# f4ah6o/duckdb.mbt

Measured on NVIDIA B200. Metric: datachunk_to_arrow_rows_per_s, higher is better.
Workload: dtype u8

## Files before the change

duckdb.mbt_b200/csrc/dmb_common.cuh:

```cuda
#pragma once

#include <cuda_runtime.h>
#include <stdint.h>

#include "duckdb_mb_gpu.h"

namespace dmb {

constexpr int kThreads = 256;
constexpr int kVec = DMB_VECTOR_SIZE;
constexpr int kNumSMs = 148;

void set_error(const char *fmt, ...);
int32_t check_cuda(cudaError_t e, const char *what);

struct alignas(16) i128 {
  uint64_t lo;
  int64_t hi;
};
struct alignas(16) u128 {
  uint64_t lo;
  uint64_t hi;
};
struct alignas(16) interval_t {
  int32_t months;
  int32_t days;
  int64_t micros;
};
struct alignas(16) month_day_nano_t {
  int32_t months;
  int32_t days;
  int64_t nanos;
};

template <typename T, int R>
struct alignas(sizeof(T) * R) Pack {
  T v[R];
};

template <int N>
struct RawVec;
template <>
struct RawVec<1> { using type = unsigned char; };
template <>
struct RawVec<2> { using type = unsigned short; };
template <>
struct RawVec<4> { using type = unsigned int; };
template <>
struct RawVec<8> { using type = uint2; };
template <>
struct RawVec<16> { using type = uint4; };

template <typename P>
__device__ __forceinline__ P ld_stream(const P *p) {
  using R = typename RawVec<sizeof(P)>::type;
  R r = __ldcs(reinterpret_cast<const R *>(p));
  P out;
  memcpy(&out, &r, sizeof(P));
  return out;
}
template <typename P>
__device__ __forceinline__ void st_stream(P *p, const P &v) {
  using R = typename RawVec<sizeof(P)>::type;
  R r;
  memcpy(&r, &v, sizeof(P));
  __stcs(reinterpret_cast<R *>(p), r);
}

struct BatchView {
  const uint32_t *counts;
  const int64_t *row_off;
  int64_t nchunks;
  int64_t nrows;
};

__device__ __forceinline__ int64_t find_chunk(const BatchView &b, int64_t row) {
  int64_t lo = 0, hi = b.nchunks;
  while (hi - lo > 1) {
    int64_t mid = (lo + hi) >> 1;
    if (__ldg(b.row_off + mid) <= row) lo = mid; else hi = mid;
  }
  return lo;
}

__device__ __forceinline__ uint64_t chunk_valid_bits(const uint64_t *vslab, const dmb_vec_desc *vecs,
                                                     int64_t c, int local, int take) {
  uint64_t keep = take >= 64 ? ~0ull : ((1ull << take) - 1ull);
  int64_t vo = vecs[c].val_off;
  if (vo < 0) return keep;
  const uint64_t *m = vslab + vo;
  int w = local >> 6, s = local & 63;
  uint64_t bits = __ldg(m + w) >> s;
  if (s && s + take > 64) bits |= __ldg(m + w + 1) << (64 - s);
  return bits & keep;
}

__device__ __forceinline__ uint64_t gather_valid64(const BatchView &b, const uint64_t *vslab,
                                                   const dmb_vec_desc *vecs, int64_t r0) {
  if (r0 >= b.nrows) return 0ull;
  int64_t c = find_chunk(b, r0);
  uint64_t word = 0;
  int filled = 0;
  while (filled < 64 && r0 + filled < b.nrows) {
    int64_t local = r0 + filled - __ldg(b.row_off + c);
    int64_t avail = (int64_t)__ldg(b.counts + c) - local;
    if (avail <= 0) { ++c; continue; }
    int take = (int)(avail < (int64_t)(64 - filled) ? avail : (int64_t)(64 - filled));
    word |= chunk_valid_bits(vslab, vecs, c, (int)local, take) << filled;
    filled += take;
  }
  return word;
}

__device__ __forceinline__ bool tile_is_regular(const BatchView &b, int64_t t) {
  if (t >= b.nchunks) return false;
  int64_t ro = __ldg(b.row_off + t);
  if (ro != t * (int64_t)kVec) return false;
  uint32_t cnt = __ldg(b.counts + t);
  return cnt == (uint32_t)kVec || ro + cnt == b.nrows;
}

__device__ __forceinline__ uint32_t pack8(uint64_t bytes01) {
  return (uint32_t)((bytes01 * 0x0102040810204080ull) >> 56);
}
__device__ __forceinline__ uint64_t spread8(uint32_t bits) {
  uint64_t x = (uint64_t)(bits & 0xff) * 0x0101010101010101ull;
  x &= 0x8040201008040201ull;
  x += 0x7f7f7f7f7f7f7f7full;
  return (x >> 7) & 0x0101010101010101ull;
}

struct BitSrc {
  const uint32_t *w;
  int64_t base;
};
__device__ __forceinline__ BitSrc bit_src(const uint8_t *bm, int64_t bit_offset) {
  const uintptr_t a = reinterpret_cast<uintptr_t>(bm);
  return BitSrc{reinterpret_cast<const uint32_t *>(a & ~(uintptr_t)3), bit_offset + (int64_t)(a & 3u) * 8};
}

__device__ __forceinline__ uint32_t load_bits32(const uint32_t *w, int64_t p, int take) {
  const int64_t wi = p >> 5;
  const int s = (int)(p & 31);
  const uint32_t lo = __ldg(w + wi);
  const uint32_t hi = (s + take > 32) ? __ldg(w + wi + 1) : 0u;
  const uint32_t r = __funnelshift_r(lo, hi, (uint32_t)s);
  return take >= 32 ? r : (r & ((1u << take) - 1u));
}

__device__ __forceinline__ uint4 shift_words(const uint4 &a, const uint4 &b, int ws, uint32_t sh) {
  uint32_t w0, w1, w2, w3, w4;
  switch (ws) {
    case 0: w0 = a.x; w1 = a.y; w2 = a.z; w3 = a.w; w4 = b.x; break;
    case 1: w0 = a.y; w1 = a.z; w2 = a.w; w3 = b.x; w4 = b.y; break;
    case 2: w0 = a.z; w1 = a.w; w2 = b.x; w3 = b.y; w4 = b.z; break;
    default: w0 = a.w; w1 = b.x; w2 = b.y; w3 = b.z; w4 = b.w; break;
  }
  return make_uint4(__funnelshift_r(w0, w1, sh), __funnelshift_r(w1, w2, sh), __funnelshift_r(w2, w3, sh), __funnelshift_r(w3, w4, sh));
}

template <int W>
__device__ __forceinline__ uint32_t word_keep(uint32_t bits, int i) {
  if (W >= 4) return ((bits >> (i * 4 / W)) & 1u) ? 0xffffffffu : 0u;
  if (W == 2) {
    const uint32_t b = bits >> (2 * i);
    return ((b & 1u) ? 0x0000ffffu : 0u) | ((b & 2u) ? 0xffff0000u : 0u);
  }
  const uint32_t b = bits >> (4 * i);
  return ((b & 1u) | ((b & 2u) << 7) | ((b & 4u) << 14) | ((b & 8u) << 21)) * 0xffu;
}

__device__ __forceinline__ uint4 enum_entry(const dmb_enum_job &job, uint32_t idx) {
  const uint32_t o0 = __ldg(job.dict_offsets + idx), o1 = __ldg(job.dict_offsets + idx + 1);
  const uint32_t len = o1 - o0;
  const uint8_t *q = job.dict_data + o0;
  uint4 e = make_uint4(len, 0, 0, 0);
  if (len <= 12u) {
    uint32_t w[3] = {0u, 0u, 0u};
#pragma unroll
    for (uint32_t k = 0; k < 12u; ++k)
      if (k < len) w[k >> 2] |= (uint32_t)__ldg(q + k) << (8u * (k & 3u));
    e.y = w[0]; e.z = w[1]; e.w = w[2];
  } else {
    e.y = (uint32_t)__ldg(q) | ((uint32_t)__ldg(q + 1) << 8) | ((uint32_t)__ldg(q + 2) << 16) | ((uint32_t)__ldg(q + 3) << 24);
    const uint64_t p = job.dict_host_base + o0;
    e.z = (uint32_t)p;
    e.w = (uint32_t)(p >> 32);
  }
  return e;
}


constexpr uint64_t kFlagAggregate = 1ull << 62;
constexpr uint64_t kFlagPrefix = 2ull << 62;
constexpr uint64_t kValueMask = (1ull << 62) - 1ull;
__device__ __forceinline__ uint64_t ld_status(const unsigned long long *p) {
  return *reinterpret_cast<const volatile unsigned long long *>(p);
}
__device__ __forceinline__ unsigned long long global_ns() { unsigned long long t; asm volatile("mov.u64 %0, %globaltimer;" : "=l"(t)); return t; }

constexpr unsigned long long kGroupOne = 1ull << 56;
constexpr unsigned long long kGroupSumMask = kGroupOne - 1ull;
__device__ __forceinline__ uint64_t lookback_groups(const unsigned long long *status, const unsigned long long *gsum, const unsigned long long *gpre,
                                                    int64_t tile, int lane, unsigned long long *err_flags, unsigned long long err_bit,
                                                    unsigned long long limit_ns) {
  if (tile <= 0) return 0;
  const int64_t g = tile >> 5;
  const int64_t lo = g >= 1 ? 32 * (g - 1) : 0;
  const int64_t idx0 = tile - 1 - lane, idx1 = tile - 33 - lane;
  const bool in0 = idx0 >= lo, in1 = idx1 >= lo;
  int64_t hbase = g - 2;
  uint64_t st0 = 0, st1 = 0, ga = 0, gb = 0;
  uint64_t prefix = 0;
  unsigned long long t0 = 0;
  unsigned spins = 0;
  auto give_up = [&]() -> bool {
    ++spins;
    if (spins > 8u) __nanosleep(100);
    if ((spins & 63u) != 0u && limit_ns != 0ull) return false;
    const unsigned long long now = global_ns();
    if (t0 == 0) t0 = now;
    if (__any_sync(0xffffffffu, now - t0 > limit_ns)) {
      if (lane == 0) atomicOr(err_flags, err_bit);
      return true;
    }
    return false;
  };
  {
    const int64_t h = hbase - lane;
    if (h >= 0) { ga = ld_status(gpre + h); gb = ld_status(gsum + h); }
  }
  {
    uint64_t v;
    int state;
    while (true) {
      if (in0 && (st0 >> 62) == 0) st0 = ld_status(status + idx0);
      if (in1 && (st1 >> 62) == 0) st1 = ld_status(status + idx1);
      v = 0;
      state = 0;
#pragma unroll
      for (int j = 0; j < 2; ++j) {
        const uint64_t st = j ? st1 : st0;
        const bool in = j ? in1 : in0;
        if (state == 0) {
          const uint32_t ready = __ballot_sync(0xffffffffu, !in || (st >> 62) != 0);
          const uint32_t is_p = __ballot_sync(0xffffffffu, in && (st >> 62) == 2);
          const int first_p = is_p ? (__ffs(is_p) - 1) : 31;
          const uint32_t need = first_p >= 31 ? 0xffffffffu : ((2u << first_p) - 1u);
          if ((ready & need) != need) state = 2;
          else {
            if (in && lane <= first_p) v += st & kValueMask;
            if (is_p) state = 1;
          }
        }
      }
      if (state != 2) break;
      if (give_up()) { state = 1; break; }
    }
#pragma unroll
    for (int d = 16; d > 0; d >>= 1) v += __shfl_xor_sync(0xffffffffu, v, d);
    prefix = v;
    if (state == 1) return prefix;
  }
  while (true) {
    const int64_t h = hbase - lane;
    uint32_t is_p;
    int first_p;
    while (true) {
      const bool pa = h < 0 || (ga >> 62) == 2;
      const bool cb = h >= 0 && ((gb >> 56) & 63ull) == 32ull;
      is_p = __ballot_sync(0xffffffffu, pa);
      first_p = is_p ? (__ffs(is_p) - 1) : 32;
// ... 21 lines not shown
```

duckdb.mbt_b200/csrc/kernels_fixed.cu:

```cuda

#include "dmb_common.cuh"

namespace dmb {

constexpr int kGroupU = 4;

template <typename S>
__device__ __forceinline__ int64_t to_i64(S v) { return (int64_t)v; }
template <>
__device__ __forceinline__ int64_t to_i64<uint64_t>(uint64_t v) {
  return v > 0x7fffffffffffffffull ? 0 : (int64_t)v;
}
template <>
__device__ __forceinline__ int64_t to_i64<double>(double v) {
  if (!(v >= -9223372036854775808.0 && v < 9223372036854775808.0)) return 0;
  return __double2ll_rn(v);
}
template <>
__device__ __forceinline__ int64_t to_i64<float>(float v) {
  if (!(v >= -9223372036854775808.0f && v < 9223372036854775808.0f)) return 0;
  return __float2ll_rn(v);
}
template <>
__device__ __forceinline__ int64_t to_i64<i128>(i128 v) {
// ... 59 lines not shown
  const __int128 q = (x + rounding) / power;
  return (q >= -(__int128)9223372036854775807ll - 1 && q <= (__int128)9223372036854775807ll) ? (int64_t)q : 0;
}
template <typename S>
__device__ __forceinline__ double dec_to_f64(S v, int scale) {
  const int64_t x = (int64_t)v;
  const double dp = kDoublePow10[scale < 0 ? 0 : (scale > 38 ? 38 : scale)];
  if (scale == 0 || (x <= 9007199254740992ll && x >= -9007199254740992ll)) return (double)x / dp;
  const int64_t power = pow10_i64(scale);
  return (double)(x / power) + (double)(x % power) / dp;
}
template <>
__device__ __forceinline__ double dec_to_f64<i128>(i128 v, int scale) {
  const __int128 x = as_int128(v);
  const double dp = kDoublePow10[scale < 0 ? 0 : (scale > 38 ? 38 : scale)];
  if (scale == 0 || (x <= (__int128)9007199254740992ll && x >= -(__int128)9007199254740992ll)) return int128_to_f64(x) / dp;
  const __int128 power = pow10_i128(scale);
  return int128_to_f64(x / power) + int128_to_f64(x % power) / dp;
}

template <typename S>
__device__ __forceinline__ int32_t to_i32_sat(S v) {
  int64_t x = (int64_t)v;
  return x > 2147483647ll ? 2147483647 : (x < -2147483648ll ? (int32_t)-2147483648ll : (int32_t)x);
}
template <>
__device__ __forceinline__ int32_t to_i32_sat<uint64_t>(uint64_t v) {
  return v > 2147483647ull ? 2147483647 : (int32_t)v;
}

__device__ __forceinline__ int64_t floor_div(int64_t a, int64_t b) {
  int64_t q = a / b;
  return (a % b != 0 && ((a < 0) != (b < 0))) ? q - 1 : q;
}

__device__ __forceinline__ int32_t date_ref_quirk(int32_t days) {
  int64_t z = (int64_t)days + 719468;
  int64_t era = (z >= 0 ? z : z - 146096) / 146097;
  int64_t doe = z - era * 146097;
  int64_t yoe = (doe - doe / 1460 + doe / 36524 - doe / 146096) / 365;
  int64_t y = yoe + era * 400;
  int64_t doy = doe - (365 * yoe + yoe / 4 - yoe / 100);
  int64_t mp = (5 * doy + 2) / 153;
  int64_t m = mp < 10 ? mp + 3 : mp - 9;
  if (m <= 2) y += 1;
  if (y >= 1970 || y < 1 || y > 9999) return days;
  auto leaps_before = [](int64_t yy) { return yy / 4 - yy / 100 + yy / 400; };
  int64_t missing = leaps_before(1969) - leaps_before(y - 1);
  return (int32_t)((int64_t)days + missing);
}

struct CvNoParam { __device__ __forceinline__ CvNoParam(int32_t = 0) {} };
struct CvSame : CvNoParam { using CvNoParam::CvNoParam; template <typename S> __device__ __forceinline__ S operator()(S v) const { return v; } };
struct CvI64 : CvNoParam { using CvNoParam::CvNoParam; template <typename S> __device__ __forceinline__ int64_t operator()(S v) const { return to_i64<S>(v); } };
struct CvI32Trunc : CvNoParam { using CvNoParam::CvNoParam; template <typename S> __device__ __forceinline__ int32_t operator()(S v) const { return (int32_t)to_i64<S>(v); } };
struct CvF64 : CvNoParam { using CvNoParam::CvNoParam; template <typename S> __device__ __forceinline__ double operator()(S v) const { return to_f64<S>(v); } };
struct CvBoolByte : CvNoParam { using CvNoParam::CvNoParam; template <typename S> __device__ __forceinline__ uint8_t operator()(S v) const { return nonzero<S>(v) ? 1 : 0; } };
struct CvI32Sat : CvNoParam { using CvNoParam::CvNoParam; template <typename S> __device__ __forceinline__ int32_t operator()(S v) const { return to_i32_sat<S>(v); } };
struct CvDecBase { int scale; __device__ __forceinline__ CvDecBase(int32_t p = 0) : scale(p) {} };
struct CvDecI64 : CvDecBase { using CvDecBase::CvDecBase; template <typename S> __device__ __forceinline__ int64_t operator()(S v) const { return dec_to_i64<S>(v, scale); } };
struct CvDecI32Trunc : CvDecBase { using CvDecBase::CvDecBase; template <typename S> __device__ __forceinline__ int32_t operator()(S v) const { return (int32_t)dec_to_i64<S>(v, scale); } };
struct CvDecF64 : CvDecBase { using CvDecBase::CvDecBase; template <typename S> __device__ __forceinline__ double operator()(S v) const { return dec_to_f64<S>(v, scale); } };
struct CvDecBoolByte : CvDecBase { using CvDecBase::CvDecBase; template <typename S> __device__ __forceinline__ uint8_t operator()(S v) const { return dec_to_i64<S>(v, scale) != 0 ? 1 : 0; } };
struct CvI128 : CvNoParam {
  using CvNoParam::CvNoParam;
  template <typename S> __device__ __forceinline__ i128 operator()(S v) const {
    i128 r; r.lo = (uint64_t)(int64_t)v; r.hi = (int64_t)v < 0 ? -1 : 0; return r;
  }
};
struct CvTsS : CvNoParam { using CvNoParam::CvNoParam; __device__ __forceinline__ int64_t operator()(int64_t v) const { return (int64_t)((uint64_t)v * 1000000ull); } };
struct CvTsMs : CvNoParam { using CvNoParam::CvNoParam; __device__ __forceinline__ int64_t operator()(int64_t v) const { return (int64_t)((uint64_t)v * 1000ull); } };
struct CvTsNs : CvNoParam { using CvNoParam::CvNoParam; __device__ __forceinline__ int64_t operator()(int64_t v) const { return floor_div(v, 1000); } };
struct CvMdn : CvNoParam {
  using CvNoParam::CvNoParam;
  __device__ __forceinline__ month_day_nano_t operator()(interval_t v) const {
    month_day_nano_t r; r.months = v.months; r.days = v.days; r.nanos = (int64_t)((uint64_t)v.micros * 1000ull); return r;
  }
};
struct CvDateRef : CvNoParam { using CvNoParam::CvNoParam; __device__ __forceinline__ int32_t operator()(int32_t v) const { return date_ref_quirk(v); } };
__device__ __forceinline__ int64_t ts_ref_quirk(int64_t micros) {
  const int64_t kDay = 86400000000ll;
  const int64_t days = floor_div(micros, kDay);
  if (days < -2147483648ll || days > 2147483647ll) return micros;
  const int64_t tod = micros - days * kDay;
  return (int64_t)date_ref_quirk((int32_t)days) * kDay + tod;
}
template <typename Pre>
struct CvTsRef : CvNoParam { using CvNoParam::CvNoParam; __device__ __forceinline__ int64_t operator()(int64_t v) const { return ts_ref_quirk(Pre()(v)); } };
struct CvId64 : CvNoParam { using CvNoParam::CvNoParam; __device__ __forceinline__ int64_t operator()(int64_t v) const { return v; } };

template <typename D> __device__ __forceinline__ D zero_of() { D z; memset(&z, 0, sizeof(D)); return z; }

template <typename S, typename D, typename F>
__device__ __forceinline__ void convert_chunk(const S *__restrict__ in, const uint64_t *__restrict__ mask,
                                              D *__restrict__ out, int count, F f) {
  constexpr int W = sizeof(S) > sizeof(D) ? sizeof(S) : sizeof(D);
  constexpr int R = 16 / W;
  constexpr int U = 4;
  using PS = Pack<S, R>;
  using PD = Pack<D, R>;
  const int nvec = count / R;
  const bool out_vec_ok = (reinterpret_cast<uintptr_t>(out) % sizeof(PD)) == 0;
  const PS *vin = reinterpret_cast<const PS *>(in);
  PD *vout = reinterpret_cast<PD *>(out);
  for (int base = threadIdx.x; base < nvec; base += kThreads * U) {
    PS x[U];
#pragma unroll
    for (int u = 0; u < U; ++u) {
      int v = base + u * kThreads;
      if (v < nvec) x[u] = ld_stream(vin + v);
    }
#pragma unroll
    for (int u = 0; u < U; ++u) {
      int v = base + u * kThreads;
      if (v < nvec) {
        int row = v * R;
        uint32_t bits = mask ? (uint32_t)(__ldg(mask + (row >> 6)) >> (row & 63)) : 0xffffffffu;
        PD y;
#pragma unroll
        for (int r = 0; r < R; ++r) y.v[r] = ((bits >> r) & 1u) ? (D)f(x[u].v[r]) : zero_of<D>();
        if (out_vec_ok) {
          st_stream(vout + v, y);
        } else {
#pragma unroll
          for (int r = 0; r < R; ++r) out[row + r] = y.v[r];
        }
      }
    }
  }
  for (int row = nvec * R + threadIdx.x; row < count; row += kThreads) {
    bool valid = mask ? ((__ldg(mask + (row >> 6)) >> (row & 63)) & 1ull) : true;
    out[row] = valid ? (D)f(in[row]) : zero_of<D>();
  }
}

template <typename S, typename D, typename F>
__device__ __forceinline__ void convert_group(const dmb_fixed_job &job, const BatchView &b, int64_t c0, int G, F f) {
  constexpr int W = sizeof(S) > sizeof(D) ? sizeof(S) : sizeof(D);
  constexpr int R = 16 / W;
  constexpr int U = kGroupU;
  constexpr int VPC = kVec / R;
  using PS = Pack<S, R>;
  using PD = Pack<D, R>;
  PS x[U];
  int64_t cc[U];
  int lv[U];
  bool act[U];
#pragma unroll
  for (int u = 0; u < U; ++u) {
    const int v = threadIdx.x + u * kThreads;
    const int g = v / VPC;
    lv[u] = v - g * VPC;
    cc[u] = c0 + g;
    act[u] = g < G && cc[u] < b.nchunks && (lv[u] + 1) * R <= (int)__ldg(b.counts + cc[u]);
    if (act[u]) {
      const S *in = reinterpret_cast<const S *>(reinterpret_cast<const uint8_t *>(job.in_data) + job.vecs[cc[u]].data_off);
      x[u] = ld_stream(reinterpret_cast<const PS *>(in) + lv[u]);
    }
  }
#pragma unroll
  for (int u = 0; u < U; ++u) {
    if (!act[u]) continue;
    const int64_t vo = job.vecs[cc[u]].val_off;
    const int row = lv[u] * R;
    const uint32_t bits = vo >= 0 ? (uint32_t)(__ldg(job.in_validity + vo + (row >> 6)) >> (row & 63)) : 0xffffffffu;
    D *out = reinterpret_cast<D *>(job.out_values) + __ldg(b.row_off + cc[u]);
    PD y;
#pragma unroll
    for (int r = 0; r < R; ++r) y.v[r] = ((bits >> r) & 1u) ? (D)f(x[u].v[r]) : zero_of<D>();
    if ((reinterpret_cast<uintptr_t>(out) % sizeof(PD)) == 0) {
      st_stream(reinterpret_cast<PD *>(out) + lv[u], y);
    } else {
#pragma unroll
      for (int r = 0; r < R; ++r) out[row + r] = y.v[r];
    }
  }
  for (int t = threadIdx.x; t < G * R; t += kThreads) {
    const int g = t / R;
    const int64_t c = c0 + g;
    if (c >= b.nchunks) break;
    const int count = (int)__ldg(b.counts + c);
    const int row = (count / R) * R + (t - g * R);
    if (row >= count) continue;
    const dmb_vec_desc vd = job.vecs[c];
    const S *in = reinterpret_cast<const S *>(reinterpret_cast<const uint8_t *>(job.in_data) + vd.data_off);
    const bool valid = vd.val_off >= 0 ? ((__ldg(job.in_validity + vd.val_off + (row >> 6)) >> (row & 63)) & 1ull) : true;
    D *out = reinterpret_cast<D *>(job.out_values) + __ldg(b.row_off + c);
    out[row] = valid ? (D)f(in[row]) : zero_of<D>();
  }
}

__device__ __forceinline__ void bool_bits_tile(const BatchView &b, const dmb_fixed_job &job, int64_t t) {
  const int64_t r0 = t * (int64_t)kVec + 8 * (int64_t)threadIdx.x;
  if (r0 >= b.nrows) return;
  uint8_t *out = reinterpret_cast<uint8_t *>(job.out_values) + (r0 >> 3);
  uint32_t bits;
  if (tile_is_regular(b, t)) {
    const dmb_vec_desc vd = job.vecs[t];
    const uint8_t *in = reinterpret_cast<const uint8_t *>(job.in_data) + vd.data_off;
    int local = 8 * threadIdx.x;
    uint64_t bytes = __ldcs(reinterpret_cast<const unsigned long long *>(in + local));
    bytes = (bytes | (bytes >> 1) | (bytes >> 2) | (bytes >> 3) | (bytes >> 4) | (bytes >> 5) |
             (bytes >> 6) | (bytes >> 7)) & 0x0101010101010101ull;
    bits = pack8(bytes);
    if (vd.val_off >= 0) bits &= (uint32_t)reinterpret_cast<const uint8_t *>(job.in_validity + vd.val_off)[threadIdx.x];
    int64_t left = b.nrows - r0;
    if (left < 8) bits &= (1u << left) - 1u;
  } else {
    int64_t c = find_chunk(b, r0);
    bits = 0;
    for (int k = 0; k < 8 && r0 + k < b.nrows; ++k) {
      int64_t row = r0 + k;
      while (row >= __ldg(b.row_off + c + 1)) ++c;
      int local = (int)(row - __ldg(b.row_off + c));
      const uint8_t *in = reinterpret_cast<const uint8_t *>(job.in_data) + job.vecs[c].data_off;
      bool valid = chunk_valid_bits(job.in_validity, job.vecs, c, local, 1) != 0;
      if (valid && in[local] != 0) bits |= 1u << k;
    }
  }
  *out = (uint8_t)bits;
}

__device__ __forceinline__ void validity_tile(const BatchView &b, const dmb_fixed_job &job, int64_t t,
                                              uint64_t *s_words) {
  const int64_t nwords = (b.nrows + 63) >> 6;
  const int lane = threadIdx.x & 31;
  {
    const int64_t w = t * DMB_VALIDITY_WORDS + lane;
    uint64_t word = 0;
    if (w < nwords) {
      if (tile_is_regular(b, t)) {
        int64_t vo = job.vecs[t].val_off;
        word = vo < 0 ? ~0ull : __ldcs(reinterpret_cast<const unsigned long long *>(job.in_validity + vo + lane));
        int64_t left = b.nrows - (w << 6);
        if (left < 64) word &= (1ull << left) - 1ull;
      } else {
        word = gather_valid64(b, job.in_validity, job.vecs, w << 6);
      }
      if (job.out_validity) __stcs(reinterpret_cast<unsigned long long *>(job.out_validity + w), word);
    }
    s_words[lane] = word;
    if (job.null_count) {
      int64_t left = b.nrows - (w << 6);
      int live = w < nwords ? (left < 64 ? (int)left : 64) : 0;
      int nulls = live - __popcll(word);
      nulls = __reduce_add_sync(0xffffffffu, nulls);
      if (lane == 0 && nulls) atomicAdd(job.null_count, (unsigned long long)nulls);
    }
  }
  if (job.out_valid_bytes) {
    __syncwarp();
#pragma unroll 2
    for (int g = lane; g < kVec / 8; g += 32) {
      const int64_t r0 = t * (int64_t)kVec + 8 * (int64_t)g;
      if (r0 < b.nrows) {
        uint32_t bits = reinterpret_cast<const uint8_t *>(s_words)[g];
        uint64_t bytes = spread8(bits);
        uint8_t *dst = job.out_valid_bytes + r0;
        if (r0 + 8 <= b.nrows) {
          __stcs(reinterpret_cast<unsigned long long *>(dst), bytes);
        } else {
          for (int k = 0; r0 + k < b.nrows; ++k) dst[k] = (uint8_t)(bytes >> (8 * k));
        }
      }
    }
    __syncwarp();
  }
}

enum { kKindConvert = 0, kKindBoolBits = 1, kKindValidityOnly = 2 };

template <typename S, typename D, int KIND>
struct GroupOf {
  static constexpr int W = sizeof(S) > sizeof(D) ? sizeof(S) : sizeof(D);
  static constexpr int R = 16 / W;
  static constexpr int value = KIND == kKindValidityOnly ? kThreads / 32 : ((KIND == kKindConvert && R >= 4) ? (kThreads * kGroupU) / (kVec / R) : 1);
};

template <typename S, typename D, typename F, int KIND>
__global__ void __launch_bounds__(kThreads)
fixed_batch_kernel(const dmb_fixed_job *__restrict__ jobs, int njobs, BatchView b) {
  __shared__ uint64_t s_words[kThreads / 32][DMB_VALIDITY_WORDS];
  __shared__ dmb_fixed_job s_job;
  constexpr int G = GroupOf<S, D, KIND>::value;
  const int64_t ntiles = (b.nrows + kVec - 1) / kVec;
  const int64_t groups = (b.nchunks + G - 1) / G;
  const int64_t items = (int64_t)njobs * groups;
  int cur_job = -1;
  for (int64_t item = blockIdx.x; item < items; item += gridDim.x) {
    const int j = (int)(item / groups);
    const int64_t i0 = (item - (int64_t)j * groups) * G;
    if (j != cur_job) {
      __syncthreads();
      if (threadIdx.x < sizeof(dmb_fixed_job) / 8)
        reinterpret_cast<uint64_t *>(&s_job)[threadIdx.x] = reinterpret_cast<const uint64_t *>(jobs + j)[threadIdx.x];
      __syncthreads();
      cur_job = j;
    }
    const dmb_fixed_job &job = s_job;
    if (KIND == kKindConvert && job.out_values) {
      if (G > 1) {
        convert_group<S, D, F>(job, b, i0, G, F(job.param));
      } else {
        const int count = (int)__ldg(b.counts + i0);
        if (count > 0) {
          const dmb_vec_desc vd = job.vecs[i0];
          const S *in = reinterpret_cast<const S *>(reinterpret_cast<const uint8_t *>(job.in_data) + vd.data_off);
          const uint64_t *mask = vd.val_off < 0 ? nullptr : job.in_validity + vd.val_off;
          D *out = reinterpret_cast<D *>(job.out_values) + __ldg(b.row_off + i0);
          convert_chunk<S, D, F>(in, mask, out, count, F(job.param));
        }
      }
    }
    if (KIND == kKindBoolBits) {
      for (int64_t i = i0; i < i0 + G && i < b.nchunks; ++i)
        if (i < ntiles && job.out_values) bool_bits_tile(b, job, i);
    }
    if (job.out_validity || job.out_valid_bytes || job.null_count) {
      const int warp = threadIdx.x >> 5;
      for (int64_t i = i0 + warp; i < i0 + G && i < b.nchunks && i < ntiles; i += kThreads / 32) validity_tile(b, job, i, s_words[warp]);
    }
  }
}

typedef void (*fixed_kernel_fn)(const dmb_fixed_job *, int, BatchView);

#define DMB_FOR_NUMERIC(DST, DT, CV)                                                              \
  case DMB_OP(DMB_PHYS_BOOL, DST): return fixed_batch_kernel<uint8_t, DT, CV, kKindConvert>;      \
  case DMB_OP(DMB_PHYS_I8, DST): return fixed_batch_kernel<int8_t, DT, CV, kKindConvert>;         \
  case DMB_OP(DMB_PHYS_F32, DST): return fixed_batch_kernel<float, DT, CV, kKindConvert>;         \
  case DMB_OP(DMB_PHYS_F64, DST): return fixed_batch_kernel<double, DT, CV, kKindConvert>;        \
  DMB_FOR_INTS_NO8(DST, DT, CV)

#define DMB_FOR_INTS_NO8(DST, DT, CV)                                                             \
  case DMB_OP(DMB_PHYS_I16, DST): return fixed_batch_kernel<int16_t, DT, CV, kKindConvert>;       \
  case DMB_OP(DMB_PHYS_I32, DST): return fixed_batch_kernel<int32_t, DT, CV, kKindConvert>;       \
  case DMB_OP(DMB_PHYS_I64, DST): return fixed_batch_kernel<int64_t, DT, CV, kKindConvert>;       \
  case DMB_OP(DMB_PHYS_U8, DST): return fixed_batch_kernel<uint8_t, DT, CV, kKindConvert>;        \
  case DMB_OP(DMB_PHYS_U16, DST): return fixed_batch_kernel<uint16_t, DT, CV, kKindConvert>;      \
  case DMB_OP(DMB_PHYS_U32, DST): return fixed_batch_kernel<uint32_t, DT, CV, kKindConvert>;      \
  case DMB_OP(DMB_PHYS_U64, DST): return fixed_batch_kernel<uint64_t, DT, CV, kKindConvert>;

#define DMB_FOR_DECIMAL(DST, DT, CV)                                                              \
  case DMB_OP(DMB_PHYS_I16, DST): return fixed_batch_kernel<int16_t, DT, CV, kKindConvert>;       \
  case DMB_OP(DMB_PHYS_I32, DST): return fixed_batch_kernel<int32_t, DT, CV, kKindConvert>;       \
  case DMB_OP(DMB_PHYS_I64, DST): return fixed_batch_kernel<int64_t, DT, CV, kKindConvert>;       \
  case DMB_OP(DMB_PHYS_I128, DST): return fixed_batch_kernel<i128, DT, CV, kKindConvert>;

static fixed_kernel_fn select_kernel(int32_t op) {
  switch (op) {
    case DMB_OP(DMB_PHYS_BOOL, DMB_DST_SAME):
    case DMB_OP(DMB_PHYS_I8, DMB_DST_SAME):
    case DMB_OP(DMB_PHYS_U8, DMB_DST_SAME): return fixed_batch_kernel<uint8_t, uint8_t, CvSame, kKindConvert>;
    case DMB_OP(DMB_PHYS_I16, DMB_DST_SAME):
    case DMB_OP(DMB_PHYS_U16, DMB_DST_SAME): return fixed_batch_kernel<uint16_t, uint16_t, CvSame, kKindConvert>;
    case DMB_OP(DMB_PHYS_I32, DMB_DST_SAME):
    case DMB_OP(DMB_PHYS_U32, DMB_DST_SAME):
    case DMB_OP(DMB_PHYS_F32, DMB_DST_SAME): return fixed_batch_kernel<uint32_t, uint32_t, CvSame, kKindConvert>;
    case DMB_OP(DMB_PHYS_I64, DMB_DST_SAME):
    case DMB_OP(DMB_PHYS_U64, DMB_DST_SAME):
    case DMB_OP(DMB_PHYS_F64, DMB_DST_SAME): return fixed_batch_kernel<uint64_t, uint64_t, CvSame, kKindConvert>;
    case DMB_OP(DMB_PHYS_I128, DMB_DST_SAME):
    case DMB_OP(DMB_PHYS_U128, DMB_DST_SAME):
    case DMB_OP(DMB_PHYS_INTERVAL, DMB_DST_SAME):
    case DMB_OP(DMB_PHYS_I128, DMB_DST_I128): return fixed_batch_kernel<u128, u128, CvSame, kKindConvert>;
    DMB_FOR_NUMERIC(DMB_DST_I64, int64_t, CvI64)
    case DMB_OP(DMB_PHYS_I128, DMB_DST_I64): return fixed_batch_kernel<i128, int64_t, CvI64, kKindConvert>;
    DMB_FOR_NUMERIC(DMB_DST_I32_TRUNC, int32_t, CvI32Trunc)
    case DMB_OP(DMB_PHYS_I128, DMB_DST_I32_TRUNC): return fixed_batch_kernel<i128, int32_t, CvI32Trunc, kKindConvert>;
    case DMB_OP(DMB_PHYS_U128, DMB_DST_I64): return fixed_batch_kernel<u128, int64_t, CvI64, kKindConvert>;
    case DMB_OP(DMB_PHYS_U128, DMB_DST_I32_TRUNC): return fixed_batch_kernel<u128, int32_t, CvI32Trunc, kKindConvert>;
    DMB_FOR_NUMERIC(DMB_DST_F64, double, CvF64)
    case DMB_OP(DMB_PHYS_I128, DMB_DST_F64): return fixed_batch_kernel<i128, double, CvF64, kKindConvert>;
    case DMB_OP(DMB_PHYS_U128, DMB_DST_F64): return fixed_batch_kernel<u128, double, CvF64, kKindConvert>;
    DMB_FOR_NUMERIC(DMB_DST_BOOL_BYTE, uint8_t, CvBoolByte)
    case DMB_OP(DMB_PHYS_I128, DMB_DST_BOOL_BYTE): return fixed_batch_kernel<i128, uint8_t, CvBoolByte, kKindConvert>;
    case DMB_OP(DMB_PHYS_U128, DMB_DST_BOOL_BYTE): return fixed_batch_kernel<u128, uint8_t, CvBoolByte, kKindConvert>;
    DMB_FOR_DECIMAL(DMB_DST_DEC_I64, int64_t, CvDecI64)
    DMB_FOR_DECIMAL(DMB_DST_DEC_I32_TRUNC, int32_t, CvDecI32Trunc)
    DMB_FOR_DECIMAL(DMB_DST_DEC_F64, double, CvDecF64)
    DMB_FOR_DECIMAL(DMB_DST_DEC_BOOL_BYTE, uint8_t, CvDecBoolByte)
    case DMB_OP(DMB_PHYS_BOOL, DMB_DST_BOOL_BITS): return fixed_batch_kernel<uint8_t, uint8_t, CvSame, kKindBoolBits>;
    case DMB_OP(DMB_PHYS_I16, DMB_DST_I128): return fixed_batch_kernel<int16_t, i128, CvI128, kKindConvert>;
    case DMB_OP(DMB_PHYS_I32, DMB_DST_I128): return fixed_batch_kernel<int32_t, i128, CvI128, kKindConvert>;
    case DMB_OP(DMB_PHYS_I64, DMB_DST_I128): return fixed_batch_kernel<int64_t, i128, CvI128, kKindConvert>;
    case DMB_OP(DMB_PHYS_I8, DMB_DST_I32_SAT): return fixed_batch_kernel<int8_t, int32_t, CvI32Sat, kKindConvert>;
    DMB_FOR_INTS_NO8(DMB_DST_I32_SAT, int32_t, CvI32Sat)
    case DMB_OP(DMB_PHYS_I64, DMB_DST_TS_US_FROM_S): return fixed_batch_kernel<int64_t, int64_t, CvTsS, kKindConvert>;
    case DMB_OP(DMB_PHYS_I64, DMB_DST_TS_US_FROM_MS): return fixed_batch_kernel<int64_t, int64_t, CvTsMs, kKindConvert>;
    case DMB_OP(DMB_PHYS_I64, DMB_DST_TS_US_FROM_NS): return fixed_batch_kernel<int64_t, int64_t, CvTsNs, kKindConvert>;
    case DMB_OP(DMB_PHYS_INTERVAL, DMB_DST_MONTH_DAY_NANO): return fixed_batch_kernel<interval_t, month_day_nano_t, CvMdn, kKindConvert>;
    case DMB_OP(DMB_PHYS_I32, DMB_DST_DATE_REF): return fixed_batch_kernel<int32_t, int32_t, CvDateRef, kKindConvert>;
    case DMB_OP(DMB_PHYS_I64, DMB_DST_TS_REF): return fixed_batch_kernel<int64_t, int64_t, CvTsRef<CvId64>, kKindConvert>;
    case DMB_OP(DMB_PHYS_I64, DMB_DST_TS_REF_FROM_S): return fixed_batch_kernel<int64_t, int64_t, CvTsRef<CvTsS>, kKindConvert>;
    case DMB_OP(DMB_PHYS_I64, DMB_DST_TS_REF_FROM_MS): return fixed_batch_kernel<int64_t, int64_t, CvTsRef<CvTsMs>, kKindConvert>;
    case DMB_OP(DMB_PHYS_I64, DMB_DST_TS_REF_FROM_NS): return fixed_batch_kernel<int64_t, int64_t, CvTsRef<CvTsNs>, kKindConvert>;
    case DMB_OP_VALIDITY_ONLY: return fixed_batch_kernel<uint8_t, uint8_t, CvSame, kKindValidityOnly>;
    default: return nullptr;
  }
}

__global__ void __launch_bounds__(kThreads)
valid_bytes_to_masks_kernel(const uint8_t *__restrict__ valid, uint32_t *__restrict__ out32,
                            unsigned long long *null_count, int64_t nrows) {
  const int64_t nhalf = (nrows + 31) >> 5;
  const int64_t nhalf_total = ((nrows + 63) >> 6) << 1;
  const int lane = threadIdx.x & 31;
  int64_t warp = ((int64_t)blockIdx.x * kThreads + threadIdx.x) >> 5;
  const int64_t nwarps = ((int64_t)gridDim.x * kThreads) >> 5;
  int nulls = 0;
  for (int64_t h = warp; h < nhalf_total; h += nwarps) {
    int64_t row = (h << 5) + lane;
    bool live = h < nhalf && row < nrows;
    bool v = live ? (__ldcs(valid + row) != 0) : false;
    uint32_t word = __ballot_sync(0xffffffffu, v);
    if (lane == 0) out32[h] = word;
    nulls += (live && !v) ? 1 : 0;
  }
  if (null_count) {
    nulls = __reduce_add_sync(0xffffffffu, nulls);
    if (lane == 0 && nulls) atomicAdd(null_count, (unsigned long long)nulls);
  }
}

}

using namespace dmb;

extern "C" int32_t dmb_dev_fixed_batch(const dmb_fixed_job *jobs_dev, const dmb_fixed_job *jobs_host,
                                       int32_t njobs, const uint32_t *counts, const int64_t *row_off,
                                       int64_t nchunks, int64_t nrows, void *stream) {
  if (njobs <= 0 || nchunks <= 0 || nrows <= 0) return 0;
  if (!jobs_dev || !jobs_host) { set_error("dmb_dev_fixed_batch: jobs is null"); return -1; }
  BatchView b{counts, row_off, nchunks, nrows};
  const int64_t max_grid = (int64_t)kNumSMs * 8;
  for (int32_t j0 = 0; j0 < njobs;) {
    int32_t j1 = j0 + 1;
    while (j1 < njobs && jobs_host[j1].op == jobs_host[j0].op) ++j1;
    fixed_kernel_fn fn = select_kernel(jobs_host[j0].op);
    if (!fn) { set_error("dmb_dev_fixed_batch: unsupported conversion op 0x%x (job %d)", jobs_host[j0].op, j0); return -1; }
    int group = 1;
    if (jobs_host[j0].op == DMB_OP_VALIDITY_ONLY) group = kThreads / 32;
    else if ((jobs_host[j0].op & 0xff) != DMB_DST_BOOL_BITS) {
      const int wi = dmb_phys_width(jobs_host[j0].op >> 8), wo = dmb_op_out_width(jobs_host[j0].op);
      const int w = wi > wo ? wi : wo;
      if (w > 0 && w <= 4) group = (kThreads * kGroupU) / (kVec / (16 / w));
    }
    const int64_t items = (int64_t)(j1 - j0) * ((nchunks + group - 1) / group);
    const int grid = (int)(items < max_grid ? items : max_grid);
    fn<<<grid, kThreads, 0, (cudaStream_t)stream>>>(jobs_dev + j0, j1 - j0, b);
    if (check_cuda(cudaGetLastError(), "fixed_batch_kernel launch")) return -1;
    j0 = j1;
  }
  return 0;
}

extern "C" int32_t dmb_dev_valid_bytes_to_masks(const uint8_t *valid_bytes, uint64_t *out_validity,
                                                unsigned long long *null_count, int64_t nrows,
                                                void *stream) {
  if (nrows <= 0) return 0;
  int64_t warps = (nrows + 31) / 32;
  int64_t blocks = (warps + 7) / 8;
  int64_t max_grid = (int64_t)kNumSMs * 8;
  int grid = (int)(blocks < max_grid ? blocks : max_grid);
  valid_bytes_to_masks_kernel<<<grid, kThreads, 0, (cudaStream_t)stream>>>(
      valid_bytes, reinterpret_cast<uint32_t *>(out_validity), null_count, nrows);
  return check_cuda(cudaGetLastError(), "valid_bytes_to_masks_kernel launch");
}

extern "C" int32_t dmb_op_out_width(int32_t op) {
  int phys = op >> 8, dst = op & 0xff;
  static const int phys_w[DMB_PHYS_COUNT] = {1, 1, 2, 4, 8, 1, 2, 4, 8, 4, 8, 16, 16, 16, 16};
  if (phys < 0 || phys >= DMB_PHYS_STRING) return -1;
  bool numeric = phys <= DMB_PHYS_F64;
  bool integer = phys >= DMB_PHYS_I8 && phys <= DMB_PHYS_U64;
  bool huge = phys == DMB_PHYS_I128 || phys == DMB_PHYS_U128;
  bool decimal = phys == DMB_PHYS_I16 || phys == DMB_PHYS_I32 || phys == DMB_PHYS_I64 || phys == DMB_PHYS_I128;
  switch (dst) {
    case DMB_DST_SAME: return phys_w[phys];
    case DMB_DST_I32_TRUNC: return (numeric || huge) ? 4 : -1;
    case DMB_DST_I64: return (numeric || huge) ? 8 : -1;
    case DMB_DST_F64: return (numeric || huge) ? 8 : -1;
    case DMB_DST_BOOL_BYTE: return (numeric || huge) ? 1 : -1;
    case DMB_DST_DEC_I32_TRUNC: return decimal ? 4 : -1;
    case DMB_DST_DEC_I64: return decimal ? 8 : -1;
    case DMB_DST_DEC_F64: return decimal ? 8 : -1;
    case DMB_DST_DEC_BOOL_BYTE: return decimal ? 1 : -1;
    case DMB_DST_BOOL_BITS: return phys == DMB_PHYS_BOOL ? 0 : -1;
    case DMB_DST_I128:
      return (phys == DMB_PHYS_I16 || phys == DMB_PHYS_I32 || phys == DMB_PHYS_I64 || phys == DMB_PHYS_I128) ? 16 : -1;
    case DMB_DST_I32_SAT: return integer ? 4 : -1;
    case DMB_DST_TS_US_FROM_S:
    case DMB_DST_TS_US_FROM_MS:
    case DMB_DST_TS_US_FROM_NS:
    case DMB_DST_TS_REF:
    case DMB_DST_TS_REF_FROM_S:
    case DMB_DST_TS_REF_FROM_MS:
    case DMB_DST_TS_REF_FROM_NS: return phys == DMB_PHYS_I64 ? 8 : -1;
    case DMB_DST_MONTH_DAY_NANO: return phys == DMB_PHYS_INTERVAL ? 16 : -1;
    case DMB_DST_DATE_REF: return phys == DMB_PHYS_I32 ? 4 : -1;
    default: return -1;
  }
}

extern "C" int32_t dmb_phys_width(int32_t phys) {
  static const int phys_w[DMB_PHYS_COUNT] = {1, 1, 2, 4, 8, 1, 2, 4, 8, 4, 8, 16, 16, 16, 16};
  return (phys < 0 || phys >= DMB_PHYS_COUNT) ? -1 : phys_w[phys];
}
```

Before: 15.60 billion.

## Split validity work into a separate span-based warp kernel with occupancy-sized grids

Moves validity bitmap, valid-bytes and null-count generation out of the per-op conversion kernel into one dedicated kernel. In that kernel each warp handles a span of 32 tiles and keeps several validity words in flight, with a fast path when every tile in the span is regular. Grid size now comes from the occupancy API instead of a fixed 8 CTAs per SM, and input descriptor loads are reordered so the data offset is fetched before the count check. This cuts shared memory in the conversion kernels and removes one launch per validity-only op group, but it adds an extra launch covering all jobs and an occupancy query on every call.

```diff
diff --git a/duckdb.mbt_b200/csrc/dmb_common.cuh b/duckdb.mbt_b200/csrc/dmb_common.cuh
--- a/duckdb.mbt_b200/csrc/dmb_common.cuh
+++ b/duckdb.mbt_b200/csrc/dmb_common.cuh
@@ -114,10 +114,9 @@
 
 __device__ __forceinline__ bool tile_is_regular(const BatchView &b, int64_t t) {
   if (t >= b.nchunks) return false;
-  int64_t ro = __ldg(b.row_off + t);
-  if (ro != t * (int64_t)kVec) return false;
-  uint32_t cnt = __ldg(b.counts + t);
-  return cnt == (uint32_t)kVec || ro + cnt == b.nrows;
+  const int64_t ro = __ldg(b.row_off + t);
+  const uint32_t cnt = __ldg(b.counts + t);
+  return (ro == t * (int64_t)kVec) & ((cnt == (uint32_t)kVec) | (ro + cnt == b.nrows));
 }
 
 __device__ __forceinline__ uint32_t pack8(uint64_t bytes01) {
diff --git a/duckdb.mbt_b200/csrc/kernels_fixed.cu b/duckdb.mbt_b200/csrc/kernels_fixed.cu
--- a/duckdb.mbt_b200/csrc/kernels_fixed.cu
+++ b/duckdb.mbt_b200/csrc/kernels_fixed.cu
@@ -235,16 +235,18 @@
     const int g = v / VPC;
     lv[u] = v - g * VPC;
     cc[u] = c0 + g;
-    act[u] = g < G && cc[u] < b.nchunks && (lv[u] + 1) * R <= (int)__ldg(b.counts + cc[u]);
+    act[u] = g < G && cc[u] < b.nchunks;
     if (act[u]) {
-      const S *in = reinterpret_cast<const S *>(reinterpret_cast<const uint8_t *>(job.in_data) + job.vecs[cc[u]].data_off);
-      x[u] = ld_stream(reinterpret_cast<const PS *>(in) + lv[u]);
+      const uint64_t data_off = __ldg(&job.vecs[cc[u]].data_off);
+      act[u] = (lv[u] + 1) * R <= (int)__ldg(b.counts + cc[u]);
+      const S *in = reinterpret_cast<const S *>(reinterpret_cast<const uint8_t *>(job.in_data) + data_off);
+      if (act[u]) x[u] = ld_stream(reinterpret_cast<const PS *>(in) + lv[u]);
     }
   }
 #pragma unroll
   for (int u = 0; u < U; ++u) {
     if (!act[u]) continue;
-    const int64_t vo = job.vecs[cc[u]].val_off;
+    const int64_t vo = __ldg(&job.vecs[cc[u]].val_off);
     const int row = lv[u] * R;
     const uint32_t bits = vo >= 0 ? (uint32_t)(__ldg(job.in_validity + vo + (row >> 6)) >> (row & 63)) : 0xffffffffu;
     D *out = reinterpret_cast<D *>(job.out_values) + __ldg(b.row_off + cc[u]);
@@ -304,66 +306,117 @@
   *out = (uint8_t)bits;
 }
 
-__device__ __forceinline__ void validity_tile(const BatchView &b, const dmb_fixed_job &job, int64_t t,
-                                              uint64_t *s_words) {
+__device__ __forceinline__ uint64_t tile_word(const BatchView &b, const dmb_fixed_job &job, int64_t w, bool regular, int64_t vo) {
+  if (!regular) return gather_valid64(b, job.in_validity, job.vecs, w << 6);
+  uint64_t word = vo < 0 ? ~0ull : __ldcs(reinterpret_cast<const unsigned long long *>(job.in_validity + vo + (w & (DMB_VALIDITY_WORDS - 1))));
+  const int64_t left = b.nrows - (w << 6);
+  if (left < 64) word &= (1ull << left) - 1ull;
+  return word;
+}
+
+__device__ __forceinline__ int word_nulls(const BatchView &b, int64_t w, uint64_t word) {
+  const int64_t left = b.nrows - (w << 6);
+  return (left <= 0 ? 0 : (left < 64 ? (int)left : 64)) - __popcll(word);
+}
+
+__device__ __forceinline__ void valid_bytes_tile(const BatchView &b, const dmb_fixed_job &job, int64_t t,
+                                                 const uint64_t *s_words, int lane) {
+  __syncwarp();
+#pragma unroll 2
+  for (int g = lane; g < kVec / 8; g += 32) {
+    const int64_t r0 = t * (int64_t)kVec + 8 * (int64_t)g;
+    if (r0 < b.nrows) {
+      uint32_t bits = reinterpret_cast<const uint8_t *>(s_words)[g];
+      uint64_t bytes = spread8(bits);
+      uint8_t *dst = job.out_valid_bytes + r0;
+      if (r0 + 8 <= b.nrows) {
+        __stcs(reinterpret_cast<unsigned long long *>(dst), bytes);
+      } else {
+        for (int k = 0; r0 + k < b.nrows; ++k) dst[k] = (uint8_t)(bytes >> (8 * k));
+      }
+    }
+  }
+  __syncwarp();
+}
+
+constexpr int kSpanTiles = 32;
+constexpr int kSpanInFlight = 4;
+
+__global__ void __launch_bounds__(kThreads)
+validity_kernel(const dmb_fixed_job *__restrict__ jobs, int njobs, BatchView b) {
+  __shared__ uint64_t s_words[kThreads / 32][kSpanInFlight][DMB_VALIDITY_WORDS];
+  __shared__ dmb_fixed_job s_job[kThreads / 32];
+  const int lane = threadIdx.x & 31, warp = threadIdx.x >> 5;
+  const int64_t ntiles = (b.nrows + kVec - 1) / kVec;
   const int64_t nwords = (b.nrows + 63) >> 6;
-  const int lane = threadIdx.x & 31;
-  {
-    const int64_t w = t * DMB_VALIDITY_WORDS + lane;
-    uint64_t word = 0;
-    if (w < nwords) {
-      if (tile_is_regular(b, t)) {
-        int64_t vo = job.vecs[t].val_off;
-        word = vo < 0 ? ~0ull : __ldcs(reinterpret_cast<const unsigned long long *>(job.in_validity + vo + lane));
-        int64_t left = b.nrows - (w << 6);
-        if (left < 64) word &= (1ull << left) - 1ull;
+  const int64_t spans = (ntiles + kSpanTiles - 1) / kSpanTiles;
+  const int64_t items = (int64_t)njobs * spans;
+  for (int64_t item = (int64_t)blockIdx.x * (kThreads / 32) + warp; item < items; item += (int64_t)gridDim.x * (kThreads / 32)) {
+    const int j = (int)(item / spans);
+    const int64_t t0 = (item - (int64_t)j * spans) * kSpanTiles;
+    const int nt = (int)(ntiles - t0 < kSpanTiles ? ntiles - t0 : kSpanTiles);
+    __syncwarp();
+    if (lane < (int)(sizeof(dmb_fixed_job) / 8))
+      reinterpret_cast<uint64_t *>(&s_job[warp])[lane] = __ldg(reinterpret_cast<const unsigned long long *>(jobs + j) + lane);
+    __syncwarp();
+    const dmb_fixed_job &job = s_job[warp];
+    if (!job.out_validity && !job.out_valid_bytes && !job.null_count) continue;
+    bool regular = false;
+    int64_t vo = -1;
+    if (lane < nt) {
+      vo = __ldg(&job.vecs[t0 + lane].val_off);
+      regular = tile_is_regular(b, t0 + lane);
+    }
+    int nulls = 0;
+    for (int k0 = 0; k0 < nt; k0 += kSpanInFlight) {
+      uint64_t word[kSpanInFlight];
+      if (__all_sync(0xffffffffu, regular || lane >= nt)) {
+#pragma unroll
+        for (int u = 0; u < kSpanInFlight; ++u) {
+          const int64_t vo_k = __shfl_sync(0xffffffffu, vo, k0 + u);
+          const int64_t w = (t0 + k0 + u) * DMB_VALIDITY_WORDS + lane;
+          word[u] = (k0 + u < nt && w < nwords) ? tile_word(b, job, w, true, vo_k) : 0ull;
+        }
       } else {
-        word = gather_valid64(b, job.in_validity, job.vecs, w << 6);
+#pragma unroll
+        for (int u = 0; u < kSpanInFlight; ++u) {
+          const bool reg_k = __shfl_sync(0xffffffffu, regular, k0 + u);
+          const int64_t vo_k = __shfl_sync(0xffffffffu, vo, k0 + u);
+          const int64_t w = (t0 + k0 + u) * DMB_VALIDITY_WORDS + lane;
+          word[u] = (k0 + u < nt && w < nwords) ? tile_word(b, job, w, reg_k, vo_k) : 0ull;
+        }
       }
-      if (job.out_validity) __stcs(reinterpret_cast<unsigned long long *>(job.out_validity + w), word);
-    }
-    s_words[lane] = word;
+#pragma unroll
+      for (int u = 0; u < kSpanInFlight; ++u) {
+        const int64_t w = (t0 + k0 + u) * DMB_VALIDITY_WORDS + lane;
+        if (job.out_validity && k0 + u < nt && w < nwords) __stcs(reinterpret_cast<unsigned long long *>(job.out_validity + w), word[u]);
+        nulls += word_nulls(b, w, word[u]);
+        s_words[warp][u][lane] = word[u];
+      }
+      if (job.out_valid_bytes) {
+#pragma unroll 1
+        for (int u = 0; u < kSpanInFlight && k0 + u < nt; ++u) valid_bytes_tile(b, job, t0 + k0 + u, s_words[warp][u], lane);
+      }
+    }
     if (job.null_count) {
-      int64_t left = b.nrows - (w << 6);
-      int live = w < nwords ? (left < 64 ? (int)left : 64) : 0;
-      int nulls = live - __popcll(word);
       nulls = __reduce_add_sync(0xffffffffu, nulls);
       if (lane == 0 && nulls) atomicAdd(job.null_count, (unsigned long long)nulls);
     }
   }
-  if (job.out_valid_bytes) {
-    __syncwarp();
-#pragma unroll 2
-    for (int g = lane; g < kVec / 8; g += 32) {
-      const int64_t r0 = t * (int64_t)kVec + 8 * (int64_t)g;
-      if (r0 < b.nrows) {
-        uint32_t bits = reinterpret_cast<const uint8_t *>(s_words)[g];
-        uint64_t bytes = spread8(bits);
-        uint8_t *dst = job.out_valid_bytes + r0;
-        if (r0 + 8 <= b.nrows) {
-          __stcs(reinterpret_cast<unsigned long long *>(dst), bytes);
-        } else {
-          for (int k = 0; r0 + k < b.nrows; ++k) dst[k] = (uint8_t)(bytes >> (8 * k));
-        }
-      }
-    }
-    __syncwarp();
-  }
-}
-
-enum { kKindConvert = 0, kKindBoolBits = 1, kKindValidityOnly = 2 };
+}
+
+enum { kKindConvert = 0, kKindBoolBits = 1 };
 
 template <typename S, typename D, int KIND>
 struct GroupOf {
   static constexpr int W = sizeof(S) > sizeof(D) ? sizeof(S) : sizeof(D);
   static constexpr int R = 16 / W;
-  static constexpr int value = KIND == kKindValidityOnly ? kThreads / 32 : ((KIND == kKindConvert && R >= 4) ? (kThreads * kGroupU) / (kVec / R) : 1);
+  static constexpr int value = (KIND == kKindConvert && R >= 4) ? (kThreads * kGroupU) / (kVec / R) : 1;
 };
 
 template <typename S, typename D, typename F, int KIND>
 __global__ void __launch_bounds__(kThreads)
 fixed_batch_kernel(const dmb_fixed_job *__restrict__ jobs, int njobs, BatchView b) {
-  __shared__ uint64_t s_words[kThreads / 32][DMB_VALIDITY_WORDS];
   __shared__ dmb_fixed_job s_job;
   constexpr int G = GroupOf<S, D, KIND>::value;
   const int64_t ntiles = (b.nrows + kVec - 1) / kVec;
@@ -386,11 +439,12 @@
         convert_group<S, D, F>(job, b, i0, G, F(job.param));
       } else {
         const int count = (int)__ldg(b.counts + i0);
+        const dmb_vec_desc vd = job.vecs[i0];
+        const int64_t ro = __ldg(b.row_off + i0);
         if (count > 0) {
-          const dmb_vec_desc vd = job.vecs[i0];
           const S *in = reinterpret_cast<const S *>(reinterpret_cast<const uint8_t *>(job.in_data) + vd.data_off);
           const uint64_t *mask = vd.val_off < 0 ? nullptr : job.in_validity + vd.val_off;
-          D *out = reinterpret_cast<D *>(job.out_values) + __ldg(b.row_off + i0);
+          D *out = reinterpret_cast<D *>(job.out_values) + ro;
           convert_chunk<S, D, F>(in, mask, out, count, F(job.param));
         }
       }
@@ -398,10 +452,6 @@
     if (KIND == kKindBoolBits) {
       for (int64_t i = i0; i < i0 + G && i < b.nchunks; ++i)
         if (i < ntiles && job.out_values) bool_bits_tile(b, job, i);
-    }
-    if (job.out_validity || job.out_valid_bytes || job.null_count) {
-      const int warp = threadIdx.x >> 5;
-      for (int64_t i = i0 + warp; i < i0 + G && i < b.nchunks && i < ntiles; i += kThreads / 32) validity_tile(b, job, i, s_words[warp]);
     }
   }
 }
@@ -478,7 +528,6 @@
     case DMB_OP(DMB_PHYS_I64, DMB_DST_TS_REF_FROM_S): return fixed_batch_kernel<int64_t, int64_t, CvTsRef<CvTsS>, kKindConvert>;
     case DMB_OP(DMB_PHYS_I64, DMB_DST_TS_REF_FROM_MS): return fixed_batch_kernel<int64_t, int64_t, CvTsRef<CvTsMs>, kKindConvert>;
     case DMB_OP(DMB_PHYS_I64, DMB_DST_TS_REF_FROM_NS): return fixed_batch_kernel<int64_t, int64_t, CvTsRef<CvTsNs>, kKindConvert>;
-    case DMB_OP_VALIDITY_ONLY: return fixed_batch_kernel<uint8_t, uint8_t, CvSame, kKindValidityOnly>;
     default: return nullptr;
   }
 }
@@ -516,24 +565,38 @@
   if (njobs <= 0 || nchunks <= 0 || nrows <= 0) return 0;
   if (!jobs_dev || !jobs_host) { set_error("dmb_dev_fixed_batch: jobs is null"); return -1; }
   BatchView b{counts, row_off, nchunks, nrows};
-  const int64_t max_grid = (int64_t)kNumSMs * 8;
+  auto launch = [&](fixed_kernel_fn fn, int64_t ctas, int32_t j0, int32_t n, int max_per_sm) -> int32_t {
+    int per_sm = 0;
+    if (check_cuda(cudaOccupancyMaxActiveBlocksPerMultiprocessor(&per_sm, fn, kThreads, 0), "fixed_batch occupancy")) return -1;
+    if (per_sm > max_per_sm) per_sm = max_per_sm;
+    const int64_t max_grid = (int64_t)kNumSMs * (per_sm > 0 ? per_sm : 1);
+    fn<<<(int)(ctas < max_grid ? ctas : max_grid), kThreads, 0, (cudaStream_t)stream>>>(jobs_dev + j0, n, b);
+    return check_cuda(cudaGetLastError(), "fixed_batch_kernel launch");
+  };
+  bool any_validity = false;
   for (int32_t j0 = 0; j0 < njobs;) {
     int32_t j1 = j0 + 1;
-    while (j1 < njobs && jobs_host[j1].op == jobs_host[j0].op) ++j1;
-    fixed_kernel_fn fn = select_kernel(jobs_host[j0].op);
-    if (!fn) { set_error("dmb_dev_fixed_batch: unsupported conversion op 0x%x (job %d)", jobs_host[j0].op, j0); return -1; }
-    int group = 1;
-    if (jobs_host[j0].op == DMB_OP_VALIDITY_ONLY) group = kThreads / 32;
-    else if ((jobs_host[j0].op & 0xff) != DMB_DST_BOOL_BITS) {
-      const int wi = dmb_phys_width(jobs_host[j0].op >> 8), wo = dmb_op_out_width(jobs_host[j0].op);
-      const int w = wi > wo ? wi : wo;
-      if (w > 0 && w <= 4) group = (kThreads * kGroupU) / (kVec / (16 / w));
-    }
-    const int64_t items = (int64_t)(j1 - j0) * ((nchunks + group - 1) / group);
-    const int grid = (int)(items < max_grid ? items : max_grid);
-    fn<<<grid, kThreads, 0, (cudaStream_t)stream>>>(jobs_dev + j0, j1 - j0, b);
-    if (check_cuda(cudaGetLastError(), "fixed_batch_kernel launch")) return -1;
+    const int32_t op = jobs_host[j0].op;
+    while (j1 < njobs && jobs_host[j1].op == op) ++j1;
+    for (int32_t j = j0; j < j1; ++j)
+      any_validity |= jobs_host[j].out_validity || jobs_host[j].out_valid_bytes || jobs_host[j].null_count;
+    if (op != DMB_OP_VALIDITY_ONLY) {
+      fixed_kernel_fn fn = select_kernel(op);
+      if (!fn) { set_error("dmb_dev_fixed_batch: unsupported conversion op 0x%x (job %d)", op, j0); return -1; }
+      int group = 1;
+      const int wo = dmb_op_out_width(op);
+      if ((op & 0xff) != DMB_DST_BOOL_BITS) {
+        const int wi = dmb_phys_width(op >> 8);
+        const int w = wi > wo ? wi : wo;
+        if (w > 0 && w <= 4) group = (kThreads * kGroupU) / (kVec / (16 / w));
+      }
+      if (launch(fn, (int64_t)(j1 - j0) * ((nchunks + group - 1) / group), j0, j1 - j0, wo == 16 ? 4 : INT32_MAX)) return -1;
+    }
     j0 = j1;
+  }
+  if (any_validity) {
+    const int64_t spans = ((nrows + kVec - 1) / kVec + kSpanTiles - 1) / kSpanTiles;
+    if (launch(validity_kernel, ((int64_t)njobs * spans + kThreads / 32 - 1) / (kThreads / 32), 0, njobs, INT32_MAX)) return -1;
   }
   return 0;
 }
diff --git a/profiles/fixed_batch_ab.py b/profiles/fixed_batch_ab.py
--- /dev/null
+++ b/profiles/fixed_batch_ab.py
@@ -0,0 +1,153 @@
+from __future__ import annotations
+
+import argparse
+import hashlib
+import json
+import os
+import statistics
+import subprocess
+import sys
+
+ROOT = os.path.dirname(os.path.dirname(os.path.abspath(__file__)))
+PEAK_GBS = 6455.0
+
+
+def _digest(torch, tensors) -> str:
+    h = hashlib.sha256()
+    for t in tensors:
+        n8 = t.numel() // 8 * 8
+        v = t[:n8].view(torch.int64)
+        idx = torch.arange(v.numel(), device=v.device, dtype=torch.int64) | 1
+        h.update(repr((int(v.sum().item()), int((v * idx).sum().item()), t[n8:].cpu().tolist())).encode())
+    return h.hexdigest()[:16]
+
+
+def worker(reps: int) -> dict:
+    sys.path.insert(0, ROOT)
+    import torch
+    from duckdb_mbt_b200 import chunks as ch
+    from duckdb_mbt_b200 import devgen
+
+    dev = torch.device("cuda:0")
+    torch.cuda.set_device(dev)
+    flush = torch.zeros(256 << 20, dtype=torch.uint8, device=dev)
+
+    def gen(seed):
+        g = torch.Generator(device=dev)
+        g.manual_seed(seed)
+        return g
+
+    n2 = 60_000_000
+    c2 = devgen.GeneratedBatch(n2, dev)
+    g = gen(20260103)
+    for nm in ("l_orderkey", "l_partkey", "l_suppkey", "l_linenumber"):
+        c2.add_fixed(ch.T_INTEGER, 0, g, 0.0, nm, lo=0, hi=2**31 - 1)
+    for nm in ("l_quantity", "l_extendedprice", "l_discount", "l_tax"):
+        c2.add_fixed(ch.T_DECIMAL, 15, g, 0.0, nm, lo=0, hi=10**7, dec_scale=2)
+    for nm in ("l_shipdate", "l_commitdate", "l_receiptdate"):
+        c2.add_fixed(ch.T_DATE, 0, g, 0.0, nm, lo=8035, hi=10592)
+    copy_cols = [0, 1, 2, 3, 8, 9, 10]
+    widen_cols = [4, 5, 6, 7]
+    val_cols = [0, 1, 2, 3, 4]
+    c3 = devgen.fixed_batch(100_000_000, [(ch.T_INTEGER, 0)], null_frac=0.10, seed=20260104, device=dev)
+    cols4 = [(ch.T_TIMESTAMP, 0)] * 22 + [(ch.T_DECIMAL, 18)] * 21 + [(ch.T_HUGEINT, 0)] * 21
+    c4 = devgen.fixed_batch(10_000_000, cols4, null_frac=0.30, seed=20260105, device=dev)
+    for c in c4.batch.columns:
+        if c.type_id == ch.T_DECIMAL:
+            c.dec_scale = 3
+
+    def dst(col):
+        return ch.D_I128 if col.type_id in (ch.T_DECIMAL, ch.T_HUGEINT) else ch.D_SAME
+
+    cases = {
+        "c2_copy": (c2, [(j, ch.D_SAME) for j in copy_cols]),
+        "c2_widen": (c2, [(j, ch.D_I128) for j in widen_cols]),
+        "c2_validity": (c2, [(j, ch.OP_VALIDITY_ONLY) for j in val_cols]),
+        "c2_fixed": (c2, [(j, dst(c2.batch.columns[j])) for j in copy_cols + widen_cols] + [(j, ch.OP_VALIDITY_ONLY) for j in val_cols]),
+        "c3_validity": (c3, [(0, ch.OP_VALIDITY_ONLY)]),
+        "c4": (c4, [(j, dst(c)) for j, c in enumerate(c4.batch.columns)]),
+    }
+    out = {"cases": {}}
+    for name, (db, specs) in cases.items():
+        plan = db.plan_fixed(specs, bitmap=True)
+        for _ in range(5):
+            db.run_fixed(plan)
+        torch.cuda.synchronize()
+        for o in plan[0]:
+            o.null_count.zero_()
+        db.run_fixed(plan)
+        torch.cuda.synchronize()
+        bufs = [t for o in plan[0] for t in (o.values, o.bitmap, o.null_count) if t is not None]
+        digest = _digest(torch, bufs)
+        ms = []
+        for _ in range(reps):
+            flush.add_(1)
+            e0, e1 = torch.cuda.Event(enable_timing=True), torch.cuda.Event(enable_timing=True)
+            e0.record()
+            db.run_fixed(plan)
+            e1.record()
+            torch.cuda.synchronize()
+            ms.append(e0.elapsed_time(e1))
+        alg = db.alg_bytes_fixed(plan)
+        out["cases"][name] = {"ms": statistics.median(ms), "alg_bytes": alg, "digest": digest,
+                              "launches": len({o.op for o in plan[0]})}
+        del plan, bufs
+    return out
+
+
+def gpu_info() -> str:
+    try:
+        return subprocess.run(["nvidia-smi", "--query-gpu=name,power.limit,clocks.sm,clocks.max.sm", "--format=csv,noheader", "-i", "0"],
+                              capture_output=True, text=True, timeout=30).stdout.strip()
+    except Exception as e:
+        return f"unavailable ({e})"
+
+
+def main():
+    ap = argparse.ArgumentParser()
+    ap.add_argument("--libs", nargs="+")
+    ap.add_argument("--passes", type=int, default=3)
+    ap.add_argument("--reps", type=int, default=30)
+    ap.add_argument("--out")
+    ap.add_argument("--worker", action="store_true")
+    args = ap.parse_args()
+    if args.worker:
+        print(json.dumps(worker(args.reps)), flush=True)
+        return
+    if not args.libs:
+        ap.error("--libs is required")
+    info = {"gpu_before": gpu_info()}
+    runs = {lib: [] for lib in args.libs}
+    for p in range(args.passes):
+        for lib in args.libs:
+            env = dict(os.environ, DMB_LIB_PATH=os.path.abspath(lib))
+            r = subprocess.run([sys.executable, os.path.abspath(__file__), "--worker", "--reps", str(args.reps)],
+                               env=env, capture_output=True, text=True, cwd=ROOT)
+            if r.returncode != 0:
+                sys.stderr.write(r.stderr)
+                raise SystemExit(f"worker for {lib} failed")
+            runs[lib].append(json.loads(r.stdout.strip().splitlines()[-1]))
+            print(f"pass {p} {lib}: " + ", ".join(f"{k} {v['ms']:.4f}" for k, v in runs[lib][-1]["cases"].items()), flush=True)
+    info["gpu_after"] = gpu_info()
+    summary = {"info": info, "passes": args.passes, "reps": args.reps, "peak_gbs": PEAK_GBS, "libs": {}}
+    for lib, rs in runs.items():
+        per = {}
+        for case in rs[0]["cases"]:
+            ms = [r["cases"][case]["ms"] for r in rs]
+            alg = rs[0]["cases"][case]["alg_bytes"]
+            med = statistics.median(ms)
+            per[case] = {"ms": round(med, 4), "min": round(min(ms), 4), "max": round(max(ms), 4),
+                         "of_peak": round(alg / 1e6 / med / PEAK_GBS, 4), "alg_bytes": alg,
+                         "launches": rs[0]["cases"][case]["launches"],
+                         "digests": sorted({r["cases"][case]["digest"] for r in rs})}
+        summary["libs"][lib] = per
+    text = json.dumps(summary, indent=1)
+    print(text)
+    if args.out:
+        os.makedirs(os.path.dirname(os.path.abspath(args.out)), exist_ok=True)
+        with open(args.out, "w") as f:
+            f.write(text + "\n")
+
+
+if __name__ == "__main__":
+    main()
```

After: 16.01 billion (median of 6 runs). 2.6% higher.
